# konnpaku-youmu/Model_Predictive_Control

Measured on AMD Instinct MI355X. Metric: QP solves/sec (batch, horizon N=20) at 1/2/4/8 MI355X; max|u-u_ref|, higher is better.
Workload: dtype f64; 1 GPU; cfg2: per-instance condense + box QP, FHC.py double integrator (ts=0.5), N=20, |u|<=1, x0~U(-10,10)^2; horizon=20, nx=2, nu=1, mode=fused, batch_per_gpu=4096, parallelism=dp1, graph=True, graph_steps=8, config=2

## Files before the change

model_predictive_control_amd/csrc/gi_box_core.hpp:

```cpp
#pragma once
#include <type_traits>

#include "quad.hpp"

namespace mpcqp {

template <int BS>
struct BoxOcc {
  static constexpr int w = BS <= 3 ? 4 : (BS <= 5 ? 2 : 1);
};

#ifndef MPCQP_KEYED_REDUCE
#define MPCQP_KEYED_REDUCE 1
#endif
template <class Mat>
struct QKeyed {
  static constexpr bool v = false;
};
template <int BS>
struct QKeyed<QSym<double, BS>> {
  static constexpr bool v = MPCQP_KEYED_REDUCE != 0;
};

template <class Mat>
// ... 7 lines not shown
  static constexpr int oZ = oUb + NV;
  static constexpr int oEnd = oZ + (QKeyed<Mat>::v ? NV : 0);
};

template <typename T>
__device__ __forceinline__ T bound_scale(T bnd) {
  return finite(bnd) ? T(1) / (T(1) + fabs(bnd)) : __builtin_nan("");
}

template <typename T, int RO>
struct QBounds {
  T lo[RO], hi[RO], sl[RO], su[RO];
  __device__ __forceinline__ void load(const int (&mi)[RO], const T* lbs, const T* ubs) {
#pragma unroll
    for (int s = 0; s < RO; ++s) {
      lo[s] = lbs[mi[s]];
      hi[s] = ubs[mi[s]];
      sl[s] = bound_scale(lo[s]);
      su[s] = bound_scale(hi[s]);
    }
  }
};

constexpr int key_bits(int nmax) {
  int b = 0;
  while ((1 << b) < nmax) ++b;
  return b;
}
template <int KB>
struct Key {
  static constexpr long long MASK = (1ll << KB) - 1;
  static __device__ __forceinline__ double clear(double v) {
    return __longlong_as_double(__double_as_longlong(v) & ~MASK);
  }
  static __device__ __forceinline__ double pack(double v, int code) {
    return __longlong_as_double((__double_as_longlong(v) & ~MASK) | (long long)(unsigned)code);
  }
  static __device__ __forceinline__ int code(double key) {
    return (int)(__double_as_longlong(key) & MASK);
  }
  static __device__ __forceinline__ double big() {
    return __longlong_as_double(0x7fefffffffffffffll & ~MASK);
  }
};
#ifndef MPCQP_KEY_BARE
#define MPCQP_KEY_BARE 1
#endif
__device__ __forceinline__ double key_max(double a, double b) {
#if MPCQP_KEY_BARE
  double r;
  asm("v_max_f64 %0, %1, %2" : "=v"(r) : "v"(a), "v"(b));
  return r;
#else
  return fmax(a, b);
#endif
}
__device__ __forceinline__ double key_min(double a, double b) {
#if MPCQP_KEY_BARE
  double r;
  asm("v_min_f64 %0, %1, %2" : "=v"(r) : "v"(a), "v"(b));
  return r;
#else
  return fmin(a, b);
#endif
}
template <bool MAX, int CTRL>
__device__ __forceinline__ void key_step(double& key) {
  const double o = dpp<CTRL>(key);
  key = MAX ? key_max(key, o) : key_min(key, o);
}

#ifndef MPCQP_ROW_OWNER
#define MPCQP_ROW_OWNER 1
#endif
template <class Mat>
struct QRowOwned {
  static constexpr bool v = false;
};
template <typename T, int BS>
struct QRowOwned<QSym<T, BS>> {
  static constexpr bool v = MPCQP_ROW_OWNER != 0;
};

template <class Mat_, bool OWN_ROWS = QRowOwned<Mat_>::v, bool KEY = true>
struct RowOwn {
  using Mat = Mat_;
  static constexpr bool OWNED = false;
  static constexpr bool KEYED = false;
  static constexpr int BS = Mat::RPL;
  static constexpr int RO = BS;
  static __device__ __forceinline__ bool has(const Mat&, int) { return true; }
  static __device__ __forceinline__ int row(const Mat& M, int s) { return M.bi * BS + s; }
  static __device__ __forceinline__ int mrow(const Mat& M, int s) { return M.bi * BS + s; }
  template <bool MAX, typename T, typename... P>
  static __device__ __forceinline__ void arg(T& v, int& idx, P&... pay) {
    Mat::template rows_arg<MAX>(v, idx, pay...);
  }
  template <typename T>
  static __device__ __forceinline__ T column(Mat& M, int k, T* gb, T (&colr)[BS],
                                             T (&colc)[Mat::NC], T (&cown)[RO]) {
    const T d = M.column(k, gb, colr, colc);
#pragma unroll
    for (int r = 0; r < BS; ++r) cown[r] = colr[r];
    return d;
  }
  template <typename T>
  static __device__ __forceinline__ void matvec(Mat& M, const T (&w)[RO], T* gb, T (&out)[RO]) {
    M.matvec(w, gb, out);
  }
};

template <class Mat_, bool KEY>
struct RowOwn<Mat_, true, KEY> {
  using Mat = Mat_;
  static constexpr bool OWNED = true;
  static constexpr int BS = Mat::RPL;
  static constexpr int RO = Mat::RO;
  static __device__ __forceinline__ bool has(const Mat& M, int s) { return M.owns(s); }
  static __device__ __forceinline__ int row(const Mat& M, int s) {
    return M.owns(s) ? M.bi * BS + M.own_row(s) : -1;
  }
  static __device__ __forceinline__ int mrow(const Mat& M, int s) {
    return M.bi * BS + M.own_mrow(s);
  }
  template <typename X>
  static __device__ __forceinline__ void deal(const Mat& M, const X (&full)[BS], X pad,
                                              X (&own)[RO]) {
#pragma unroll
    for (int s = 0; s < RO; ++s) {
      own[s] = pad;
#pragma unroll
      for (int j = 0; j < 4; ++j)
        if (4 * s + j < BS) own[s] = (M.bj == j) ? full[4 * s + j] : own[s];
    }
  }
  template <typename X>
  static __device__ __forceinline__ void gather(const Mat&, const X (&own)[RO], X (&full)[BS]) {
#pragma unroll
    for (int r = 0; r < BS; ++r) {
      const X v = own[r / 4];
      full[r] = (r % 4 == 0)   ? quad_lane<0>(v)
                : (r % 4 == 1) ? quad_lane<1>(v)
                : (r % 4 == 2) ? quad_lane<2>(v)
                               : quad_lane<3>(v);
    }
  }
  template <bool MAX, typename T, typename... P>
  static __device__ __forceinline__ void arg(T& v, int& idx, P&... pay) {
    Mat::template group_arg<MAX>(v, idx, pay...);
  }
  static constexpr bool KEYED = KEY && QKeyed<Mat>::v;
  using K = Key<key_bits(Mat::NMAX)>;
  template <bool MAX>
  static __device__ __forceinline__ void key_arg(double& key) {
    key_step<MAX, 0xB1>(key);
    key_step<MAX, 0x4E>(key);
    key_step<MAX, 0x124>(key);
    key_step<MAX, 0x128>(key);
  }
  template <typename T>
  static __device__ __forceinline__ T column(Mat& M, int k, T* gb, T (&colr)[BS],
                                             T (&colc)[Mat::NC], T (&cown)[RO]) {
    return M.column(k, gb, colr, colc, cown);
  }
  template <typename T>
  static __device__ __forceinline__ void matvec(Mat& M, const T (&w)[RO], T* gb, T (&out)[RO]) {
    M.matvec_own(w, gb, out);
  }
};

template <bool OWNED, class A, class B>
__device__ __forceinline__ auto& own_or_full(A& own, B& full) {
  if constexpr (OWNED) return own;
  else return full;
}


template <typename T>
__device__ __forceinline__ T mu_rate(int st, T cs, T sgn) {
  return ((st == 1) ? -cs : ((st == 2) ? cs : T(0))) * sgn;
}

template <class Own, typename T>
struct SelCmp {
  static constexpr int RO = Own::RO;
  const int (&ri)[RO];
  __device__ __forceinline__ SelCmp(const int (&ri_)[RO], const int (&)[RO], T*) : ri(ri_) {}
  __device__ __forceinline__ void scan(const int (&st)[RO], const T (&zr)[RO],
                                       const QBounds<T, RO>& B, T& viol, int& pi, T& zv) const {
    viol = -Lim<T>::inf();
    pi = 0;
    zv = T(0);
#pragma unroll
    for (int r = 0; r < RO; ++r) {
      const T vl = (B.lo[r] - zr[r]) * B.sl[r];
      const T vu = (zr[r] - B.hi[r]) * B.su[r];
      const T v = (st[r] == 0) ? fmax(vl, vu) : -Lim<T>::inf();
      const bool take = v > viol;
      viol = take ? v : viol;
      pi = take ? ri[r] : pi;
      zv = take ? zr[r] : zv;
    }
    Own::template arg<true>(viol, pi, zv);
  }
  __device__ __forceinline__ bool release(const int (&st)[RO], const T (&mu)[RO], T tol,
                                          int& k) const {
    T mv = Lim<T>::inf();
#pragma unroll
    for (int r = 0; r < RO; ++r) {
      const bool a = (st[r] == 1 || st[r] == 2) && mu[r] < -tol;
      const bool take = a && mu[r] < mv;
      mv = take ? mu[r] : mv;
      k = take ? ri[r] : k;
    }
    Own::template arg<false>(mv, k);
    return mv < Lim<T>::inf();
  }
  __device__ __forceinline__ void ratio(const int (&st)[RO], const T (&mu)[RO],
                                        const T (&co)[RO], T rm, T sgn, T& ti, int& k) const {
    ti = Lim<T>::inf();
#pragma unroll
    for (int r = 0; r < RO; ++r) {
      const T dmu = mu_rate(st[r], co[r] * rm, sgn);
      const bool cand = (st[r] == 1 || st[r] == 2) && dmu < T(0);
      const T t = cand ? -mu[r] * fast_rcp(dmu) : Lim<T>::inf();
      const bool take = t < ti;
      ti = take ? t : ti;
      k = take ? ri[r] : k;
    }
    Own::template arg<false>(ti, k);
  }
  template <class Mat>
  __device__ __forceinline__ void publish(const Mat&, const T (&)[RO]) const {}
  __device__ __forceinline__ T pivot_z(int, T zv) const { return zv; }
};

template <class Own>
struct SelKey {
  static constexpr int RO = Own::RO;
  using Mat = typename Own::Mat;
  using K = typename Own::K;
  int mi[RO], cmax[RO];
  double* zs;
  __device__ __forceinline__ SelKey(const int (&)[RO], const int (&mi_)[RO], double* gb)
      : zs(gb + BoxLds<Mat>::oZ) {
#pragma unroll
    for (int r = 0; r < RO; ++r) {
      mi[r] = mi_[r];
      cmax[r] = int(K::MASK) - mi_[r];
    }
  }
  __device__ __forceinline__ void scan(const int (&st)[RO], const double (&zr)[RO],
                                       const QBounds<double, RO>& B, double& viol, int& pi,
                                       double&) const {
    double key = -K::big();
#pragma unroll
    for (int r = 0; r < RO; ++r) {
      const double vl = (B.lo[r] - zr[r]) * B.sl[r];
      const double vu = (zr[r] - B.hi[r]) * B.su[r];
      const double v = fmin(fmax(fmax(vl, vu), -K::big()), K::big());
      key = key_max(key, K::pack((st[r] == 0) ? v : -K::big(), cmax[r]));
    }
    Own::template key_arg<true>(key);
    viol = K::clear(key);
    pi = int(K::MASK) - K::code(key);
  }
  __device__ __forceinline__ bool release(const int (&st)[RO], const double (&mu)[RO],
                                          double tol, int& k) const {
    double key = K::big();
#pragma unroll
    for (int r = 0; r < RO; ++r) {
      const bool a = (st[r] == 1 || st[r] == 2) && mu[r] < -tol;
      key = key_min(key, K::pack(a ? fmax(mu[r], -K::big()) : K::big(), cmax[r]));
    }
    Own::template key_arg<false>(key);
    k = int(K::MASK) - K::code(key);
    return K::clear(key) < K::big();
  }
  __device__ __forceinline__ void ratio(const int (&st)[RO], const double (&mu)[RO],
                                        const double (&co)[RO], double rm, double sgn,
                                        double& ti, int& k) const {
    double key = K::big();
#pragma unroll
    for (int r = 0; r < RO; ++r) {
      const double dmu = mu_rate(st[r], co[r] * rm, sgn);
      const bool cand = (st[r] == 1 || st[r] == 2) && dmu < 0.0;
      const double t = cand ? fmin(-mu[r] * fast_rcp(dmu), K::big()) : K::big();
      key = key_min(key, K::pack(t, mi[r]));
    }
    Own::template key_arg<false>(key);
    ti = K::clear(key);
    k = K::code(key);
  }
  __device__ __forceinline__ void publish(const Mat& M, const double (&zr)[RO]) const {
#pragma unroll
    for (int r = 0; r < RO; ++r)
      if (Own::has(M, r)) zs[mi[r]] = zr[r];
  }
  __device__ __forceinline__ double pivot_z(int p, double) const { return zs[p]; }
};

template <bool WARM, class Own_ = void, class Mat, typename T>
__device__ __forceinline__ int gi_box_st(Mat& M, T* gb, const T* fs, const T* lbs,
                                         const T* ubs, int n, int max_iter, T tol, bool live,
                                         T (&zfull)[Mat::RPL], int& iters,
                                         int (&stfull)[Mat::RPL] MPCQP_CLK_PARAM) {
  using Own = std::conditional_t<std::is_void_v<Own_>, RowOwn<Mat>, Own_>;
  static_assert(std::is_same_v<typename Own::Mat, Mat>, "policy of another layout");
  constexpr int BS = Mat::RPL, NC = Mat::NC;
  constexpr int RO = Own::RO;
  int ri[RO], mi[RO];
#pragma unroll
  for (int r = 0; r < RO; ++r) {
    ri[r] = Own::row(M, r);
    mi[r] = Own::mrow(M, r);
  }
  QBounds<T, RO> B;
  B.load(mi, lbs, ubs);
  const std::conditional_t<Own::KEYED, SelKey<Own>, SelCmp<Own, T>> sel(ri, mi, gb);
  T zown[Own::OWNED ? RO : 1], mu[RO];
  int stown[Own::OWNED ? RO : 1];
  auto& zr = own_or_full<Own::OWNED>(zown, zfull);
  auto& st = own_or_full<Own::OWNED>(stown, stfull);
  if constexpr (WARM && Own::OWNED) Own::deal(M, stfull, 3, stown);
#pragma unroll
  for (int r = 0; r < RO; ++r) {
    if constexpr (!WARM) st[r] = (Own::has(M, r) && ri[r] < n) ? 0 : 3;
    mu[r] = T(0);
    zr[r] = T(0);
  }
  iters = 0;
  int code = MPCQP_STATUS_OPTIMAL;
  auto refresh = [&]() {
    T w[RO], s[RO];
#pragma unroll
    for (int r = 0; r < RO; ++r) {
      const T zA = (st[r] == 1) ? B.lo[r] : ((st[r] == 2) ? B.hi[r] : T(0));
      w[r] = (st[r] == 0) ? fs[mi[r]] : -zA;
      zr[r] = zA;
    }
    Own::matvec(M, w, gb, s);
#pragma unroll
    for (int r = 0; r < RO; ++r) {
      const T g = fs[mi[r]] - s[r];
      zr[r] = (st[r] == 0) ? s[r] : zr[r];
      mu[r] = (st[r] == 1) ? g : ((st[r] == 2) ? -g : T(0));
    }
    sel.publish(M, zr);
  };
  refresh();
  bool active = live;
  if constexpr (WARM) {
    bool drop = live;
    while (true) {
      int k = 0;
      const bool found = sel.release(st, mu, tol, k);
      drop = drop && found;
      if (!__any(drop)) break;
      if (drop && ++iters > max_iter) {
        code = MPCQP_STATUS_MAXITER;
        drop = false;
        active = false;
      }
      T kr[BS], kc[NC];
      const T d = M.column(k, gb, kr, kc);
      if (drop && !(d > T(0))) {
        code = MPCQP_STATUS_NOT_CONVEX;
        drop = false;
        active = false;
      }
      if (drop) {
        M.sweep_col(k, T(1), d, kr, kc);
#pragma unroll
        for (int r = 0; r < RO; ++r)
          if (ri[r] == k) st[r] = 0;
      }
      refresh();
    }
  }
  for (int pass = 0; pass < 3; ++pass) {
    bool need_p = true;
    int p = 0, side = 1;
    T tgt = T(0), zp = T(0), gp = T(0);
    T a_viol = T(0), a_zv = T(0);
    int a_pi = 0;
    bool have_scan = false;
    while (true) {
      if (__any(active && need_p)) {
        T viol, zv = T(0);
        int pi;
        if (have_scan) {
          viol = a_viol;
          pi = a_pi;
          zv = a_zv;
        } else {
          sel.scan(st, zr, B, viol, pi, zv);
        }
        if (active && need_p) {
          if (!(viol > tol)) {
            active = false;
          } else {
            p = pi;
            const T lbp = lbs[p], ubp = ubs[p];
            zp = sel.pivot_z(p, zv);
            side = (zp < lbp) ? 1 : 2;
            tgt = (side == 1) ? lbp : ubp;
            gp = T(0);
            need_p = false;
          }
        }
      }
      MPCQP_PHASE(5);
      if (!__any(active)) break;
      bool stepping = active;
      if (stepping && ++iters > max_iter) {
        code = MPCQP_STATUS_MAXITER;
        active = false;
        stepping = false;
      }
      T c[BS], cc[NC], co[RO];
      const T mpp = Own::column(M, p, gb, c, cc, co);
      const T rm = fast_rcp(mpp);
      const T sgn = (tgt > zp) ? T(1) : T(-1);
      const T t2 = fabs(tgt - zp);
      T ti;
      int k = 0;
      sel.ratio(st, mu, co, rm, sgn, ti, k);
      const bool partial = ti < t2;
      const T s_eff = stepping ? (partial ? ti : t2) : T(0);
#pragma unroll
      for (int r = 0; r < RO; ++r) {
        const T cs = co[r] * rm;
        zr[r] = (st[r] == 0) ? fma(sgn * s_eff, cs, zr[r]) : zr[r];
        mu[r] = fma(s_eff, mu_rate(st[r], cs, sgn), mu[r]);
      }
      gp = fma(-sgn * s_eff, rm, gp);
      zp = fma(sgn, s_eff, zp);
      MPCQP_PHASE(6);
      const int idx = partial ? k : p;
      const T sigma = partial ? T(1) : T(-1);
      T kr[BS], kcol[NC];
      T d = mpp;
      if (__any(stepping && partial)) {
        d = M.column(idx, gb, kr, kcol);
      } else {
#pragma unroll
        for (int r = 0; r < BS; ++r) kr[r] = c[r];
#pragma unroll
        for (int r = 0; r < NC; ++r) kcol[r] = cc[r];
      }
      const bool bad = stepping && (partial ? !(d > T(0)) : !(d < T(0)));
      if (stepping && !bad) {
#pragma unroll
        for (int r = 0; r < RO; ++r) {
          const int i = ri[r];
          if (partial && i == k) {
            st[r] = 0;
            mu[r] = T(0);
          }
          if (!partial && i == p) {
            st[r] = side;
            zr[r] = tgt;
            mu[r] = (side == 1) ? gp : -gp;
          }
        }
        need_p = !partial;
      }
      if (bad) {
        code = MPCQP_STATUS_NOT_CONVEX;
        active = false;
      }
      sel.publish(M, zr);
      sel.scan(st, zr, B, a_viol, a_pi, a_zv);
      have_scan = true;
      if (stepping && !bad) M.sweep_col(idx, sigma, d, kr, kcol);
      MPCQP_PHASE(7);
    }
    refresh();
    T viol, zv = T(0);
    int pi;
    sel.scan(st, zr, B, viol, pi, zv);
    active = live && code == MPCQP_STATUS_OPTIMAL && viol > tol;
    if (!__any(active)) break;
  }
#pragma unroll
  for (int r = 0; r < RO; ++r) {
    zr[r] = fmin(fmax(zr[r], B.lo[r]), B.hi[r]);
  }
  if constexpr (Own::OWNED) {
    Own::gather(M, zown, zfull);
    Own::gather(M, stown, stfull);
  }
  return code;
}

template <class Own = void, class Mat, typename T>
__device__ __forceinline__ int gi_box(Mat& M, T* gb, const T* fs, const T* lbs, const T* ubs,
                                      int n, int max_iter, T tol, bool live,
                                      T (&zr)[Mat::RPL], int& iters MPCQP_CLK_PARAM) {
  int st[Mat::RPL];
  return gi_box_st<false, Own>(M, gb, fs, lbs, ubs, n, max_iter, tol, live, zr, iters,
                               st MPCQP_CLK_ARG);
}

template <typename T, int BS>
__device__ __forceinline__ int gi_box_core(Sym2D<T, BS>& M, T* buf, const T* fs, const T* lbs,
                                           const T* ubs, int n, int max_iter, T tol,
                                           T (&zr)[BS], int& iters) {
#ifdef MPCQP_PHASE_TIMING
  PhaseClock mpcqp_clk;
#endif
  return gi_box(M, buf, fs, lbs, ubs, n, max_iter, tol, true, zr, iters MPCQP_CLK_ARG);
}

}
```

model_predictive_control_amd/csrc/loop_box.hip:

```cpp
#include <type_traits>

#include "box_vjp_core.hpp"
#include "gi_box_core.hpp"
#include "quad_api.hpp"

namespace mpcqp {

template <typename T>
struct LoopArgs {
  int batch, nx, nu, N, n, steps;
  const T* H; int64_t sH;
  const T* F; int64_t sF;
  const T* A; int64_t sA;
  const T* B; int64_t sB;
  const T* x0; int64_t sX0;
  const T* lb; int64_t slb;
  const T* ub; int64_t sub;
  T* xs;
  T* us;
  T* zs;
  int32_t* status;
  int max_iter;
  T tol;
};

template <typename T>
struct LoopAffineArgs : LoopArgs<T> {
  const T* g; int64_t sG, gT;
  const T* w;
  int cold;
};

template <typename T, bool AFFINE>
using LoopArgsOf = std::conditional_t<AFFINE, LoopAffineArgs<T>, LoopArgs<T>>;

template <typename T, int NX, int NU, int BS>
struct LoopLds {
  using Box = BoxLds<QSym<T, BS>>;
  static constexpr int NMAX = 4 * BS;
  static constexpr int PMAX = NMAX * (NMAX + 1) / 2;
  static constexpr int oP = Box::oEnd;
  static constexpr int oF = oP + PMAX;
  static constexpr int oA = oF + NMAX * NX;
  static constexpr int oB = oA + NX * NX;
  static constexpr int oX = oB + NX * NU;
  static constexpr int oU = oX + NX;
  static constexpr int oS = oU + NU;
  static constexpr int size = oS + NMAX;
};

template <typename T, int BS>
struct LoopOcc {
  static constexpr int w = BS <= 2 ? 4 : 1;
};

template <typename T, int NX, int NU, int BS, bool AFFINE>
struct LoopKeyed {
  static constexpr bool v = !(sizeof(T) == 8 && NX == 4 && NU == 2 && BS == 5 && AFFINE);
};

template <typename T>
using GlobalPtr = const __attribute__((address_space(1))) T*;
template <typename T>
__device__ __forceinline__ GlobalPtr<T> sbase(const T* p) {
  const unsigned long long v = (unsigned long long)p;
  const unsigned lo = (unsigned)__builtin_amdgcn_readfirstlane((int)(v & 0xffffffffull));
  const unsigned hi = (unsigned)__builtin_amdgcn_readfirstlane((int)(v >> 32));
  return (GlobalPtr<T>)(((unsigned long long)hi << 32) | lo);
}

template <typename T>
__device__ __forceinline__ T at_bytes(GlobalPtr<T> base, unsigned bytes) {
  return *(GlobalPtr<T>)((const __attribute__((address_space(1))) char*)base + bytes);
}

template <typename T>
__device__ __forceinline__ void put_at(T* base, int64_t row, unsigned off, T v) {
  const unsigned long long p = (unsigned long long)(base + row);
  const unsigned lo = (unsigned)__builtin_amdgcn_readfirstlane((int)(p & 0xffffffffull));
  const unsigned hi = (unsigned)__builtin_amdgcn_readfirstlane((int)(p >> 32));
  asm volatile("" : "+v"(off));
  *(__attribute__((address_space(1))) T*)((__attribute__((address_space(1))) char*)(
        ((unsigned long long)hi << 32) | lo) + off * (unsigned)sizeof(T)) = v;
}

template <typename T, int NX, int NU, int BS, bool AFFINE = false>
__global__ __launch_bounds__(64, (LoopOcc<T, BS>::w)) void box_loop_kernel(
    LoopArgsOf<T, AFFINE> a) {
  using Lq = LoopLds<T, NX, NU, BS>;
  using Box = BoxLds<QSym<T, BS>>;
  constexpr int NMAX = Lq::NMAX;
  extern __shared__ __attribute__((aligned(16))) char smem_raw[];
  const int lane = threadIdx.x, g = lane >> 4, q = lane & 15;
  const int b = blockIdx.x * 4 + g;
  [[maybe_unused]] const int64_t b0 = (int64_t)blockIdx.x * 4;
  const bool live = b < a.batch;
  const int bl = live ? b : 0;
  const int n = a.n, nx = a.nx, nu = a.nu, P = n * (n + 1) / 2;
  T* gs = reinterpret_cast<T*>(smem_raw) + g * Lq::size;
  T* gb = gs + Box::oBuf;
  T* fs = gs + Box::oF;
  T* lbs = gs + Box::oLb;
  T* ubs = gs + Box::oUb;
  T* Ps = gs + Lq::oP;
  T* Fs = gs + Lq::oF;
  T* As = gs + Lq::oA;
  T* Bs = gs + Lq::oB;
  T* xg = gs + Lq::oX;
  T* ug = gs + Lq::oU;
  T* sg = gs + Lq::oS;

  {
    const T* Hb = a.H + (int64_t)bl * a.sH;
    for (int e = q; e < Lq::PMAX; e += 16) Ps[e] = e < P ? Hb[e] : T(0);
    const T* Fb = a.F + (int64_t)bl * a.sF;
    for (int e = q; e < NMAX * NX; e += 16) {
      const int i = e / NX, j = e - i * NX;
      Fs[e] = (i < n && j < nx) ? Fb[i * nx + j] : T(0);
    }
    for (int e = q; e < NX * NX; e += 16) {
      const int i = e / NX, j = e - i * NX;
      As[e] = (i < nx && j < nx) ? a.A[(int64_t)bl * a.sA + i * nx + j] : T(0);
    }
    for (int e = q; e < NX * NU; e += 16) {
      const int i = e / NU, j = e - i * NU;
      Bs[e] = (i < nx && j < nu) ? a.B[(int64_t)bl * a.sB + i * nu + j] : T(0);
    }
    if (q < NX) xg[q] = q < nx ? a.x0[(int64_t)bl * a.sX0 + q] : T(0);
  }
  bool nonfinite = false, badbox = false;
  for (int i = q; i < NMAX; i += 16) {
    const bool v = live && i < n;
    const T li = (v && a.lb) ? a.lb[(int64_t)b * a.slb + i] : -Lim<T>::inf();
    const T ui = (v && a.ub) ? a.ub[(int64_t)b * a.sub + i] : Lim<T>::inf();
    lbs[i] = li;
    ubs[i] = ui;
    badbox |= v && (!(li <= ui) || li == Lim<T>::inf() || ui == -Lim<T>::inf());
  }
  __syncthreads();
  for (int e = q; e < P; e += 16) nonfinite |= live && !finite(Ps[e]);
  for (int e = q; e < NMAX * NX; e += 16) nonfinite |= live && !finite(Fs[e]);
// ... 10 lines not shown
  M.init(lane);
  int st[BS];
#pragma unroll
  for (int r = 0; r < BS; ++r) st[r] = (M.bi * BS + r < n) ? 0 : 3;
  int failed = MPCQP_STATUS_OPTIMAL;
  int okst[BS];
#pragma unroll
  for (int r = 0; r < BS; ++r) {
    const int i = M.bi * BS + r;
    okst[r] = (lbs[i] > -Lim<T>::inf() ? 1 : 0) | (ubs[i] < Lim<T>::inf() ? 2 : 0);
  }

  constexpr bool WPACK = BS <= 2;
  [[maybe_unused]] T gn0 = T(0), gn1 = T(0), wn = T(0);
  [[maybe_unused]] auto fetch_g = [&](int t) {
    if constexpr (AFFINE) {
      if (live && a.g) {
        const auto gt = sbase(a.g + (int64_t)t * a.gT + b0 * a.sG);
        unsigned o = a.sG ? (unsigned)(g * n + q) : (unsigned)q;
        asm volatile("" : "+v"(o));
        if (q < n) gn0 = at_bytes(gt, o * (unsigned)sizeof(T));
        if constexpr (NMAX > 16)
          if (q + 16 < n) gn1 = at_bytes(gt, (o + 16u) * (unsigned)sizeof(T));
      }
    }
  };
  [[maybe_unused]] auto fetch_w = [&](int t) {
    if constexpr (AFFINE) {
      const int j = WPACK ? q - 8 : q;
      if (live && a.w && j >= 0 && j < nx) {
        const auto wt = sbase(a.w + ((int64_t)t * a.batch + b0) * nx);
        unsigned o = (unsigned)(g * nx + j);
        asm volatile("" : "+v"(o));
        (WPACK ? gn0 : wn) = at_bytes(wt, o * (unsigned)sizeof(T));
      }
    }
  };
  if constexpr (AFFINE)
    if (a.steps > 0) {
      fetch_g(0);
      fetch_w(0);
    }

  for (int t = 0; t < a.steps; ++t) {
    if constexpr (AFFINE) {
      if (live && q < nx) put_at(a.xs, ((int64_t)t * a.batch + b0) * nx, (unsigned)(g * nx + q), xg[q]);
    } else {
      if (live && q < nx) a.xs[((int64_t)t * a.batch + b) * nx + q] = xg[q];
    }
    bool nfx = false;
#pragma unroll
    for (int j = 0; j < NX; ++j) nfx |= !finite(xg[j]);
    if constexpr (AFFINE) {
#ifdef MPCQP_BOX_LOOP_PLAIN_LOAD
      if (t > 0) fetch_g(t);
#endif
      nfx |= (__ballot((!finite(gn0) && !(WPACK && q >= 8)) || !finite(gn1)) & gmask) != 0;
    }
    for (int i = q; i < NMAX; i += 16) {
      T s = T(0);
#pragma unroll
      for (int j = 0; j < NX; ++j) s = fma(Fs[i * NX + j], xg[j], s);
      if constexpr (AFFINE) s += i < 16 ? gn0 : gn1;
      fs[i] = s;
    }
    lds_exchange();
#ifndef MPCQP_BOX_LOOP_PLAIN_LOAD
    if constexpr (AFFINE)
      if (t + 1 < a.steps) fetch_g(t + 1);
#endif
    bool nf = false;
    M.load_packed(Ps, n, nf);
    const unsigned fmask = free_row_mask(M, st, g);
    int code = nfx ? MPCQP_STATUS_NONFINITE : code0;
    if (failed != MPCQP_STATUS_OPTIMAL) code = failed;
    const int sweeps = __popc(fmask);
    const bool okp = sweep_free_rows(M, gb, fmask, [&](int k, T d, const T(&colr)[BS],
                                                       const T(&colc)[BS]) {
      M.sweep_col(k, T(1), d, colr, colc);
    });
    if (code == MPCQP_STATUS_OPTIMAL && !okp) code = MPCQP_STATUS_NOT_CONVEX;
    T zr[BS];
    int iters = 0;
    using Own = RowOwn<QSym<T, BS>, QRowOwned<QSym<T, BS>>::v, LoopKeyed<T, NX, NU, BS, AFFINE>::v>;
    const int c2 = gi_box_st<true, Own>(M, gb, fs, lbs, ubs, n, a.max_iter, a.tol,
                                        live && code == MPCQP_STATUS_OPTIMAL, zr, iters,
                                        st MPCQP_CLK_ARG);
    if (code == MPCQP_STATUS_OPTIMAL) code = c2;
    const bool okc = code == MPCQP_STATUS_OPTIMAL || code == MPCQP_STATUS_MAXITER;
    if (!okc) {
      failed = code;
#pragma unroll
      for (int r = 0; r < BS; ++r) zr[r] = __builtin_nan("");
    }
    if (M.bj == 0) {
#pragma unroll
      for (int r = 0; r < BS; ++r) {
        const int i = M.bi * BS + r;
        if (i < NU) ug[i] = zr[r];
        if (i < NMAX) sg[i] = (T)st[r];
        if constexpr (AFFINE) {
          if (live && a.zs && i < n)
            put_at(a.zs, ((int64_t)t * a.batch + b0) * n, (unsigned)(g * n + i), zr[r]);
        } else {
          if (live && a.zs && i < n) a.zs[((int64_t)t * a.batch + b) * n + i] = zr[r];
        }
      }
    }
    const int word = (code & 0xff) | (((iters + sweeps) & 0xffff) << 8);
    if constexpr (AFFINE) {
      if (live && q == 0) put_at(a.status, (int64_t)t * a.batch + b0, (unsigned)g, (int32_t)word);
    } else {
      if (live && q == 0) a.status[(int64_t)t * a.batch + b] = word;
    }
    lds_exchange();
    if constexpr (AFFINE) {
      if (live && q < nu) put_at(a.us, ((int64_t)t * a.batch + b0) * nu, (unsigned)(g * nu + q), ug[q]);
    } else {
      if (live && q < nu) a.us[((int64_t)t * a.batch + b) * nu + q] = ug[q];
    }
    T xn = T(0);
    if (q < NX) {
#pragma unroll
      for (int j = 0; j < NX; ++j) xn = fma(As[q * NX + j], xg[j], xn);
#pragma unroll
      for (int j = 0; j < NU; ++j) xn = fma(Bs[q * NU + j], ug[j], xn);
    }
#ifdef MPCQP_BOX_LOOP_PLAIN_LOAD
    if constexpr (AFFINE)
      if (t > 0) fetch_w(t);
#endif
    if constexpr (AFFINE) xn += WPACK ? dpp<0x128>(gn0) : wn;
#ifndef MPCQP_BOX_LOOP_PLAIN_LOAD
    if constexpr (AFFINE)
      if (t + 1 < a.steps) fetch_w(t + 1);
#endif
#pragma unroll
    for (int r = 0; r < BS; ++r) {
      const int i = M.bi * BS + r;
      const int src = i + nu < n ? i + nu : i;
      const int s = okc ? ((int)sg[src] & okst[r]) : 0;
      if constexpr (AFFINE)
        st[r] = i < n && !a.cold ? s : (i < n ? 0 : 3);
      else
        st[r] = i < n ? s : 3;
    }
    lds_exchange();
    if (q < NX) xg[q] = xn;
    lds_exchange();
  }
  if constexpr (AFFINE) {
    if (live && q < nx)
      put_at(a.xs, ((int64_t)a.steps * a.batch + b0) * nx, (unsigned)(g * nx + q), xg[q]);
  } else {
    if (live && q < nx) a.xs[((int64_t)a.steps * a.batch + b) * nx + q] = xg[q];
  }
}

template <typename T, int NX, int NU, int BS, bool AFFINE>
static int launch_loop(const LoopArgsOf<T, AFFINE>& a, hipStream_t st) {
  using Lq = LoopLds<T, NX, NU, BS>;
  const size_t bytes = (size_t)4 * Lq::size * sizeof(T);
  if (bytes > 64 * 1024) {
    hipError_t e = hipFuncSetAttribute((const void*)box_loop_kernel<T, NX, NU, BS, AFFINE>,
                                       hipFuncAttributeMaxDynamicSharedMemorySize, (int)bytes);
    if (e != hipSuccess) return hip_fail(e, "hipFuncSetAttribute(box_loop)");
  }
// ... 95 lines not shown
```

model_predictive_control_amd/csrc/quad.hpp:

```cpp
#pragma once
#include "sym2d.hpp"

namespace mpcqp {

template <typename T>
__device__ __forceinline__ T quad_sum(T v) {
  v += dpp<0xB1>(v);
  v += dpp<0x4E>(v);
  return v;
}
template <int J, typename X>
__device__ __forceinline__ X quad_lane(X v) {
  return dpp<J | (J << 2) | (J << 4) | (J << 6)>(v);
}

template <typename T, int BS>
struct QSym {
  static constexpr int NMAX = 4 * BS;
  static constexpr int NV = NMAX;
  static constexpr int NC = BS;
  static constexpr int RPL = BS;
  static constexpr int CBUF = NMAX * BS;
  static constexpr int BUF = CBUF + NMAX;
  T m[BS][BS];
  int bi, bj;

  __device__ __forceinline__ void init(int lane) {
    const int q = lane & 15;
    bi = q >> 2;
    bj = q & 3;
  }

  template <bool MAX, typename... P>
  static __device__ __forceinline__ void rows_arg(T& v, int& idx, P&... pay) {
    arg_step<MAX, Dpp<0x124>>(v, idx, pay...);
    arg_step<MAX, Dpp<0x128>>(v, idx, pay...);
  }
  template <bool MAX, typename... P>
  static __device__ __forceinline__ void group_arg(T& v, int& idx, P&... pay) {
    arg_step<MAX, Dpp<0xB1>>(v, idx, pay...);
    arg_step<MAX, Dpp<0x4E>>(v, idx, pay...);
    rows_arg<MAX>(v, idx, pay...);
  }

  __device__ __forceinline__ void load_dense_sym(const T* D, int ld, int n) {
#pragma unroll
    for (int r = 0; r < BS; ++r)
#pragma unroll
      for (int c = 0; c < BS; ++c) {
        const int i = bi * BS + r, j = bj * BS + c;
        m[r][c] = (i < n && j < n) ? T(0.5) * (D[i * ld + j] + D[j * ld + i]) : T(0);
      }
  }

  __device__ __forceinline__ void load_packed(const T* Ps, int n, bool& nonfinite) {
#pragma unroll
    for (int r = 0; r < BS; ++r)
#pragma unroll
      for (int c = 0; c < BS; ++c) {
        const int i = bi * BS + r, j = bj * BS + c;
        T v = T(0);
        if (i < n && j < n) {
          const int idx = (j <= i) ? i * (i + 1) / 2 + j : j * (j + 1) / 2 + i;
          v = Ps[idx];
          nonfinite |= !finite(v);
        }
        m[r][c] = v;
      }
  }

  static constexpr int RO = (BS + 3) / 4;
  __device__ __forceinline__ int own_row(int s) const { return 4 * s + bj; }
  __device__ __forceinline__ bool owns(int s) const { return own_row(s) < BS; }
  __device__ __forceinline__ int own_mrow(int s) const {
    return own_row(s) < BS ? own_row(s) : BS - 1;
  }

  __device__ __forceinline__ T column(int k, T* gb, T (&colr)[BS], T (&colc)[BS]) {
    T unused[RO];
    return column(k, gb, colr, colc, unused);
  }
  __device__ __forceinline__ T column(int k, T* gb, T (&colr)[BS], T (&colc)[BS],
                                      T (&cown)[RO]) {
    const int kb = k / BS, kc = k - kb * BS;
    if (bj == kb) {
#pragma unroll
      for (int r = 0; r < BS; ++r)
#pragma unroll
        for (int c = 0; c < BS; ++c) gb[(bi * BS + r) * BS + c] = m[r][c];
    }
    lds_exchange();
#pragma unroll
    for (int r = 0; r < BS; ++r) colr[r] = gb[(bi * BS + r) * BS + kc];
#pragma unroll
    for (int c = 0; c < BS; ++c) colc[c] = gb[(bj * BS + c) * BS + kc];
#pragma unroll
    for (int s = 0; s < RO; ++s) cown[s] = gb[(bi * BS + own_mrow(s)) * BS + kc];
    const T d = gb[k * BS + kc];
    lds_exchange();
    return d;
  }

  __device__ __forceinline__ void sweep_col(int k, T sigma, T d, const T (&colr)[BS],
                                            const T (&colc)[BS]) {
    const T rd = fast_rcp(d);
    T a[BS], scol[BS], srow[BS];
    bool ik[BS], jk[BS];
#pragma unroll
    for (int r = 0; r < BS; ++r) {
      a[r] = colr[r] * rd;
      scol[r] = sigma * a[r];
      ik[r] = (bi * BS + r == k);
    }
#pragma unroll
    for (int c = 0; c < BS; ++c) {
      jk[c] = (bj * BS + c == k);
      srow[c] = jk[c] ? -rd : sigma * colc[c] * rd;
    }
#pragma unroll
    for (int r = 0; r < BS; ++r)
#pragma unroll
      for (int c = 0; c < BS; ++c) {
        const T gen = fma(-a[r], colc[c], m[r][c]);
        m[r][c] = ik[r] ? srow[c] : (jk[c] ? scol[r] : gen);
      }
  }

  __device__ __forceinline__ T sweep(int k, T sigma, T* gb) {
    T colr[BS], colc[BS];
    const T d = column(k, gb, colr, colc);
    sweep_col(k, sigma, d, colr, colc);
    return d;
  }

  __device__ __forceinline__ void matvec(const T (&w)[BS], T* gb, T (&out)[BS]) {
    T* wb = gb + CBUF;
    if (bj == 0) {
#pragma unroll
      for (int r = 0; r < BS; ++r) wb[bi * BS + r] = w[r];
    }
    lds_exchange();
    T wc[BS];
#pragma unroll
    for (int c = 0; c < BS; ++c) wc[c] = wb[bj * BS + c];
#pragma unroll
    for (int r = 0; r < BS; ++r) {
      T s = T(0);
#pragma unroll
      for (int c = 0; c < BS; ++c) s = fma(m[r][c], wc[c], s);
      out[r] = quad_sum(s);
    }
    lds_exchange();
  }

  __device__ __forceinline__ void matvec_own(const T (&w)[RO], T* gb, T (&out)[RO]) {
    T* wb = gb + CBUF;
#pragma unroll
    for (int s = 0; s < RO; ++s)
      if (owns(s)) wb[bi * BS + own_row(s)] = w[s];
    lds_exchange();
    T wc[BS];
#pragma unroll
    for (int c = 0; c < BS; ++c) wc[c] = wb[bj * BS + c];
#pragma unroll
    for (int s = 0; s < RO; ++s) out[s] = T(0);
#pragma unroll
    for (int r = 0; r < BS; ++r) {
      T s = T(0);
#pragma unroll
      for (int c = 0; c < BS; ++c) s = fma(m[r][c], wc[c], s);
      s = quad_sum(s);
      out[r / 4] = (bj == r % 4) ? s : out[r / 4];
    }
    lds_exchange();
  }
};

}
```

model_predictive_control_amd/csrc/quad_box.hip:

```cpp
#include "mpc_factor.hpp"
#include "gi_box_core.hpp"
#include "quad_api.hpp"

namespace mpcqp {

template <typename T, int BS>
struct QuadOcc {
  static constexpr int w = sizeof(T) == 8 ? (BS <= 3 ? 4 : (BS == 4 ? 3 : (BS == 5 ? 2 : 1)))
                                           : (BS <= 3 ? 4 : (BS <= 5 ? 3 : 2));
};

template <typename T, int BS>
__global__ __launch_bounds__(64, (QuadOcc<T, BS>::w)) void box_quad_kernel(BoxArgsQ<T> a) {
#ifdef MPCQP_PHASE_TIMING
  PhaseClock mpcqp_clk;
#endif
  using L = BoxLds<QSym<T, BS>>;
  constexpr int NMAX = L::NMAX;
  constexpr int PMAX = NMAX * (NMAX + 1) / 2;
  constexpr int GSZ = L::oEnd + PMAX;
  extern __shared__ __attribute__((aligned(16))) char smem_raw[];
  const int lane = threadIdx.x, g = lane >> 4, q = lane & 15;
  const int b = blockIdx.x * 4 + g;
  const bool live = b < a.batch;
// ... 1 lines not shown
  const int n = a.n, P = n * (n + 1) / 2;
  T* gs = reinterpret_cast<T*>(smem_raw) + g * GSZ;
  T* gb = gs + L::oBuf;
  T* fs = gs + L::oF;
  T* lbs = gs + L::oLb;
  T* ubs = gs + L::oUb;
  T* Ps = gs + L::oEnd;
  {
    constexpr int MAXT = (PMAX + 15) / 16;
    const T* Hb = a.H + (int64_t)bl * a.sH;
    T tmp[MAXT];
#pragma unroll
    for (int t = 0; t < MAXT; ++t) {
      const int e = q + 16 * t;
      tmp[t] = (e < P) ? Hb[e] : T(0);
    }
#pragma unroll
    for (int t = 0; t < MAXT; ++t) {
      const int e = q + 16 * t;
      if (e < P) Ps[e] = tmp[t];
    }
  }
  bool nonfinite = false, badbox = false;
  for (int i = q; i < NMAX; i += 16) {
    const bool v = live && i < n;
    const T fi = v ? a.f[(int64_t)b * a.sf + i] : T(0);
    const T li = (v && a.lb) ? a.lb[(int64_t)b * a.slb + i] : -Lim<T>::inf();
    const T ui = (v && a.ub) ? a.ub[(int64_t)b * a.sub + i] : Lim<T>::inf();
    fs[i] = fi;
    lbs[i] = li;
    ubs[i] = ui;
    nonfinite |= v && !finite(fi);
    badbox |= v && (!(li <= ui) || li == Lim<T>::inf() || ui == -Lim<T>::inf());
  }
  __syncthreads();
  QSym<T, BS> M;
  M.init(lane);
  M.load_packed(Ps, n, nonfinite);
  const unsigned long long gmask = 0xFFFFull << (16 * g);
  const bool g_nonfinite = (__ballot(nonfinite) & gmask) != 0;
  const bool g_badbox = (__ballot(badbox) & gmask) != 0;
  int code = MPCQP_STATUS_OPTIMAL;
  if (g_nonfinite) code = MPCQP_STATUS_NONFINITE;
  else if (g_badbox) code = MPCQP_STATUS_INFEASIBLE;
  bool ok = true;
  for (int k = 0; k < n; ++k) {
    const T d = M.sweep(k, T(1), gb);
    ok &= d > T(0);
  }
  if (code == MPCQP_STATUS_OPTIMAL && !ok) code = MPCQP_STATUS_NOT_CONVEX;
  T zr[BS];
  int iters = 0;
  const int c2 = gi_box(M, gb, fs, lbs, ubs, n, a.max_iter, a.tol,
                        live && code == MPCQP_STATUS_OPTIMAL, zr, iters MPCQP_CLK_ARG);
  if (code == MPCQP_STATUS_OPTIMAL) code = c2;
  if (code != MPCQP_STATUS_OPTIMAL && code != MPCQP_STATUS_MAXITER) {
#pragma unroll
    for (int r = 0; r < BS; ++r) zr[r] = __builtin_nan("");
  }
  if (live && M.bj == 0) {
#pragma unroll
    for (int r = 0; r < BS; ++r) {
      const int i = M.bi * BS + r;
      if (i < n) a.z[(int64_t)b * n + i] = zr[r];
    }
  }
  if (live && q == 0) a.status[b] = (code & 0xff) | ((iters & 0xffff) << 8);
}

template <typename T, int NX, int NU, int BS>
struct QMpcRows {
  static constexpr bool v = NX <= 2 && !(sizeof(T) == 8 && NU == 2 && BS <= 3);
};

template <typename T, int NX, int NU, class Mat>
struct QMpcOwned {
  static constexpr bool v =
      QRowOwned<Mat>::v && !(sizeof(T) == 8 && NX == 4 && NU == 2 && Mat::RPL == 5);
};

template <typename T, int NX, int NU, class Mat>
struct QMpcKeyed {
  static constexpr bool v = !(sizeof(T) == 8 && NX == 4 && NU == 2 && Mat::RPL == 4);
};

template <typename T, int NX, int NU, class Mat>
struct QMpcLds {
  static constexpr bool ROWS = QMpcRows<T, NX, NU, Mat::RPL>::v;
  int oA, oB, oQ, oQf, oR, oC, oX0, oK, oSi, oAcl, oX, oW, total, ld;
  __host__ __device__ QMpcLds(int N, int n, int tv) {
    const int S = tv ? N : 1;
    const int N2 = ROWS ? 0 : N;
    oA = BoxLds<Mat>::oEnd;
    oB = oA + S * NX * NX;
    oQ = oB + S * NX * NU;
    oQf = oQ + NX * NX;
    oR = oQf + NX * NX;
    oC = oR + NU * NU;
    oX0 = oC + N * NX;
    oK = oX0 + NX;
    oSi = oK + N2 * NU * NX;
    oAcl = oSi + N2 * NU * NU;
    oX = oAcl + N2 * NX * NX;
    oW = oX + (ROWS ? 0 : (N + 1) * NX);
    ld = Mat::NV + 1;
    total = (oW + n * ld + 1) & ~1;
  }
};

template <typename T, int NX, int NU>
__device__ __forceinline__ void load_sq(const T* s, T (&m)[NX][NU], int ld) {
#pragma unroll
  for (int i = 0; i < NX; ++i)
#pragma unroll
    for (int j = 0; j < NU; ++j) m[i][j] = s[i * ld + j];
}

template <typename T, int NX, int BS>
struct QMpcOcc {
  static constexpr int w = NX <= 2 ? QuadOcc<T, BS>::w : (QuadOcc<T, BS>::w < 2 ? 1 : 2);
};

#ifdef MPCQP_WAVE_CLOCK
constexpr int kWaveClockMax = 16384;
__device__ unsigned long long mpcqp_wave_clock[3 * kWaveClockMax];
#endif

template <typename T, int NX, int NU, class Mat, int GL, int OCC>
__global__ __launch_bounds__(64, OCC) void mpc_group_kernel(MpcArgsQ<T> a) {
#ifdef MPCQP_WAVE_CLOCK
  const unsigned long long wclk0 = __builtin_amdgcn_s_memrealtime();
#endif
  using BL = BoxLds<Mat>;
  constexpr int NV = BL::NV;
  constexpr int RPL = Mat::RPL;
  constexpr int GPW = kWave / GL;
  extern __shared__ __attribute__((aligned(16))) char smem_raw[];
  const int lane = threadIdx.x, g = lane / GL, q = lane % GL;
  const int b = blockIdx.x * GPW + g;
  const bool live = b < a.batch;
  const int bl = live ? b : 0;
  const int nx = a.nx, nu = a.nu, N = a.N, n = N * nu, tv = a.tv;
  const int S = tv ? N : 1;
  const QMpcLds<T, NX, NU, Mat> L(N, n, tv);
  T* sm = reinterpret_cast<T*>(smem_raw) + g * L.total;
  T* gb = sm + BL::oBuf;
  T* fs = sm + BL::oF;
  T* lbs = sm + BL::oLb;
  T* ubs = sm + BL::oUb;
  T* As = sm + L.oA;
  T* Bs = sm + L.oB;
  T* Qs = sm + L.oQ;
  T* Qfs = sm + L.oQf;
  T* Rs = sm + L.oR;
  T* Cs = sm + L.oC;
  T* X0s = sm + L.oX0;
  constexpr bool ROWS = QMpcRows<T, NX, NU, RPL>::v;
  [[maybe_unused]] T* Ks = sm + L.oK;
  [[maybe_unused]] T* Sis = sm + L.oSi;
  [[maybe_unused]] T* Acls = sm + L.oAcl;
  [[maybe_unused]] T* Xs = sm + L.oX;
  T* Wt = sm + L.oW;
  const int ld = L.ld;

#ifdef MPCQP_PHASE_TIMING
  PhaseClock mpcqp_clk;
// ... 440 lines not shown
#pragma unroll
          for (int ch = 0; ch < NCH; ++ch) {
            const bool at = t == cj[ch];
            T v[NU], u[NU], xn[NX];
#pragma unroll
            for (int i = 0; i < NU; ++i) {
              v[i] = at ? lj[ch][i] : T(0);
              T s = v[i];
#pragma unroll
              for (int qq = 0; qq < NX; ++qq) s = fma(Kt[i][qq], wx[ch][qq], s);
              u[i] = s;
            }
#pragma unroll
            for (int i = 0; i < NX; ++i) {
              T s = T(0);
#pragma unroll
              for (int qq = 0; qq < NX; ++qq) s = fma(Act[i][qq], wx[ch][qq], s);
#pragma unroll
              for (int qq = 0; qq < NU; ++qq) s = fma(Br[i][qq], v[qq], s);
              xn[i] = s;
            }
#pragma unroll
            for (int qq = 0; qq < NX; ++qq) wx[ch][qq] = xn[qq];
            if (cv[ch]) {
#pragma unroll
              for (int i = 0; i < NU; ++i)
                if (i < nu) Wc[ch][t * nu + i] = u[i];
            }
          }
        }
        if (q == 0) {
#pragma unroll
          for (int u = 0; u < NU; ++u) {
            T s = T(0);
#pragma unroll
            for (int qq = 0; qq < NX; ++qq) s = fma(Ba[qq][u], yk[qq], s);
            if (u < nu) fs[k * nu + u] = s;
          }
        }
        if (k > 0) {
          T yn[NX];
#pragma unroll
          for (int i = 0; i < NX; ++i) {
            T s = T(0);
#pragma unroll
            for (int qq = 0; qq < NX; ++qq) s = fma(Qr[i][qq], xnext[qq], s);
#pragma unroll
            for (int qq = 0; qq < NX; ++qq) s = fma(Ar[qq][i], yk[qq], s);
            yn[i] = s;
          }
#pragma unroll
          for (int qq = 0; qq < NX; ++qq) yk[qq] = yn[qq];
        }
#pragma unroll
        for (int i = 0; i < NU; ++i)
#pragma unroll
          for (int qq = 0; qq < NX; ++qq) Kt[i][qq] = Kn[i][qq];
#pragma unroll
        for (int i = 0; i < NX; ++i)
#pragma unroll
          for (int qq = 0; qq < NX; ++qq) Act[i][qq] = Acn[i][qq];
#pragma unroll
        for (int qq = 0; qq < NX; ++qq) xnext[qq] = xnn[qq];
      }
#pragma unroll
      for (int ch = 0; ch < NCH; ++ch)
        if (cv[ch])
          for (int i = n; i < NV; ++i) Wc[ch][i] = T(0);
    }
  }
  __syncthreads();

  MPCQP_PHASE(2);
  Mat M;
  M.init(lane);
  neg_gram<T>(M, Wt, ld, n);
  MPCQP_PHASE(3);
  for (int i = q; i < n; i += GL) nonfinite |= !finite(fs[i]);
  const unsigned long long gmask = (GL == 64 ? ~0ull : ((1ull << GL) - 1)) << (GL * g);
  if ((__ballot(nonfinite) & gmask) != 0) code = MPCQP_STATUS_NONFINITE;
  else if ((__ballot(badbox) & gmask) != 0) code = MPCQP_STATUS_INFEASIBLE;
  T zr[RPL];
  int iters = 0;
  using Own = RowOwn<Mat, QMpcOwned<T, NX, NU, Mat>::v, QMpcKeyed<T, NX, NU, Mat>::v>;
  const int c2 = gi_box<Own>(M, gb, fs, lbs, ubs, n, a.max_iter, a.tol,
                             live && code == MPCQP_STATUS_OPTIMAL, zr, iters MPCQP_CLK_ARG);
  if (code == MPCQP_STATUS_OPTIMAL) code = c2;
  MPCQP_PHASE(4);
#ifdef MPCQP_PHASE_TIMING
  mpcqp_clk.flush();
#endif
  if (code != MPCQP_STATUS_OPTIMAL && code != MPCQP_STATUS_MAXITER) {
#pragma unroll
    for (int r = 0; r < RPL; ++r) zr[r] = __builtin_nan("");
  }
  if (live && M.bj == 0) {
#pragma unroll
    for (int r = 0; r < RPL; ++r) {
      const int i = M.bi * RPL + r;
      if (i < n) a.z[(int64_t)b * n + i] = zr[r];
    }
  }
  if (live && q == 0) a.status[b] = (code & 0xff) | ((iters & 0xffff) << 8);
#ifdef MPCQP_WAVE_CLOCK
  {
    int itmax = 0;
#pragma unroll
    for (int gg = 0; gg < GPW; ++gg) {
      const int v = __builtin_amdgcn_readlane(iters, gg * GL);
      itmax = v > itmax ? v : itmax;
    }
    const unsigned long long wclk1 = __builtin_amdgcn_s_memrealtime();
    if (lane == 0 && blockIdx.x < kWaveClockMax) {
      mpcqp_wave_clock[3 * blockIdx.x] = wclk0;
      mpcqp_wave_clock[3 * blockIdx.x + 1] = wclk1;
      mpcqp_wave_clock[3 * blockIdx.x + 2] = (unsigned long long)itmax;
    }
  }
#endif
}

template <typename T, int BS>
int launch_box_quad(const BoxArgsQ<T>& a, hipStream_t st) {
  using L = BoxLds<QSym<T, BS>>;
  constexpr int NMAX = L::NMAX;
  const size_t bytes = (size_t)4 * (L::oEnd + NMAX * (NMAX + 1) / 2) * sizeof(T);
  hipLaunchKernelGGL((box_quad_kernel<T, BS>), dim3((a.batch + 3) / 4), dim3(kWave), bytes, st, a);
  MPCQP_CHECK_LAUNCH("box_quad_kernel");
  return MPCQP_OK;
}

template <typename T>
int solve_box_quad(const BoxArgsQ<T>& a, hipStream_t st) {
  return dispatch_bs<4>(a.n, [&](auto bs) {
    return launch_box_quad<T, decltype(bs)::value>(a, st);
  });
}

template <typename T, int NX, int NU, class Mat, int GL, int OCC>
int launch_mpc_group(const MpcArgsQ<T>& a, hipStream_t st) {
  constexpr int GPW = kWave / GL;
  const int n = a.N * a.nu;
  const QMpcLds<T, NX, NU, Mat> L(a.N, n, a.tv);
  const size_t bytes = (size_t)GPW * L.total * sizeof(T);
  if (bytes > 160 * 1024) {
    set_error("mpcqp_mpc_box: LDS footprint %zu B > 160 KiB", bytes);
    return MPCQP_ENOTSUP;
  }
  auto kern = mpc_group_kernel<T, NX, NU, Mat, GL, OCC>;
  if (bytes > 64 * 1024) {
    hipError_t e = hipFuncSetAttribute((const void*)kern,
                                       hipFuncAttributeMaxDynamicSharedMemorySize, (int)bytes);
    if (e != hipSuccess) return hip_fail(e, "hipFuncSetAttribute(mpc_group)");
  }
  hipLaunchKernelGGL(kern, dim3((a.batch + GPW - 1) / GPW), dim3(kWave), bytes, st, a);
  MPCQP_CHECK_LAUNCH("mpc_group_kernel");
  return MPCQP_OK;
}

template <typename T, int NX, int NU, int BS>
int launch_mpc_quad(const MpcArgsQ<T>& a, hipStream_t st) {
  return launch_mpc_group<T, NX, NU, QSym<T, BS>, 16, QMpcOcc<T, NX, BS>::w>(a, st);
}

template <typename T, int NX, int NU>
int mpc_quad_bs(const MpcArgsQ<T>& a, hipStream_t st) {
  return dispatch_bs<4>(a.N * a.nu, [&](auto bs) {
// ... 31 lines not shown
```

Measured before the change: 91.52 million solves/s.

## Add fast full-step path, prefetch next pivot bounds, defer sweep with precomputed reciprocal

Splits the dual active-set inner step into two variants. A cheap conservative filter decides whether any active constraint could block the step, and when none can, a full-step variant skips the keyed ratio reduction and the column fetch. The bounds and z value for the next pivot are prefetched right after the violation scan, and the rank-1 sweep is deferred past the branch using the already-computed reciprocal. This adds the filter's per-row work and extra live registers, and the filter tolerance could misjudge near-ties.

```diff
diff --git a/model_predictive_control_amd/csrc/gi_box_core.hpp b/model_predictive_control_amd/csrc/gi_box_core.hpp
--- a/model_predictive_control_amd/csrc/gi_box_core.hpp
+++ b/model_predictive_control_amd/csrc/gi_box_core.hpp
@@ -113,11 +113,22 @@
   static constexpr bool v = MPCQP_ROW_OWNER != 0;
 };
 
-template <class Mat_, bool OWN_ROWS = QRowOwned<Mat_>::v, bool KEY = true>
+#ifndef MPCQP_FAST_TRIP
+#define MPCQP_FAST_TRIP 1
+#endif
+#ifndef MPCQP_BOUND_AHEAD
+#define MPCQP_BOUND_AHEAD 1
+#endif
+#ifndef MPCQP_SWEEP_RD
+#define MPCQP_SWEEP_RD 1
+#endif
+
+template <class Mat_, bool OWN_ROWS = QRowOwned<Mat_>::v, bool KEY = true, bool TRIP = true>
 struct RowOwn {
   using Mat = Mat_;
   static constexpr bool OWNED = false;
   static constexpr bool KEYED = false;
+  static constexpr bool FAST = false, AHEAD = false, SWEEP_RD = false;
   static constexpr int BS = Mat::RPL;
   static constexpr int RO = BS;
   static __device__ __forceinline__ bool has(const Mat&, int) { return true; }
@@ -141,8 +152,8 @@
   }
 };
 
-template <class Mat_, bool KEY>
-struct RowOwn<Mat_, true, KEY> {
+template <class Mat_, bool KEY, bool TRIP>
+struct RowOwn<Mat_, true, KEY, TRIP> {
   using Mat = Mat_;
   static constexpr bool OWNED = true;
   static constexpr int BS = Mat::RPL;
@@ -181,6 +192,9 @@
     Mat::template group_arg<MAX>(v, idx, pay...);
   }
   static constexpr bool KEYED = KEY && QKeyed<Mat>::v;
+  static constexpr bool FAST = TRIP && (KEYED ? MPCQP_FAST_TRIP != 0 : MPCQP_FAST_TRIP == 2);
+  static constexpr bool AHEAD = TRIP && (KEYED ? MPCQP_BOUND_AHEAD != 0 : MPCQP_BOUND_AHEAD == 2);
+  static constexpr bool SWEEP_RD = FAST && MPCQP_SWEEP_RD != 0;
   using K = Key<key_bits(Mat::NMAX)>;
   template <bool MAX>
   static __device__ __forceinline__ void key_arg(double& key) {
@@ -210,6 +224,35 @@
 template <typename T>
 __device__ __forceinline__ T mu_rate(int st, T cs, T sgn) {
   return ((st == 1) ? -cs : ((st == 2) ? cs : T(0))) * sgn;
+}
+
+template <typename T>
+struct RatioFilter;
+template <>
+struct RatioFilter<double> {
+  static constexpr double DELTA = 0x1p-40, TINY = 0x1p-900;
+};
+template <>
+struct RatioFilter<float> {
+  static constexpr float DELTA = 0x1p-16f, TINY = 0x1p-100f;
+};
+template <typename T>
+__device__ __forceinline__ bool ratio_range(T t2, T huge) {
+  return t2 >= RatioFilter<T>::TINY && t2 <= huge;
+}
+template <typename T, int RO>
+__device__ __forceinline__ bool ratio_filter(const int (&st)[RO], const T (&mu)[RO],
+                                             const T (&co)[RO], T rm, T sgn, T t2) {
+  const T t2d = t2 * (T(1) + RatioFilter<T>::DELTA);
+  bool f = false;
+#pragma unroll
+  for (int r = 0; r < RO; ++r) {
+    const T dmu = mu_rate(st[r], co[r] * rm, sgn);
+    const bool cand = (st[r] == 1 || st[r] == 2) && dmu < T(0);
+    const T rhs = t2d * -dmu;
+    f = f || (cand && (mu[r] < rhs || rhs < RatioFilter<T>::TINY));
+  }
+  return f;
 }
 
 template <class Own, typename T>
@@ -261,6 +304,10 @@
     }
     Own::template arg<false>(ti, k);
   }
+  __device__ __forceinline__ bool may_block(const int (&st)[RO], const T (&mu)[RO],
+                                            const T (&co)[RO], T rm, T sgn, T t2) const {
+    return ratio_filter(st, mu, co, rm, sgn, t2) || !ratio_range(t2, Lim<T>::inf());
+  }
   template <class Mat>
   __device__ __forceinline__ void publish(const Mat&, const T (&)[RO]) const {}
   __device__ __forceinline__ T pivot_z(int, T zv) const { return zv; }
@@ -322,6 +369,11 @@
     Own::template key_arg<false>(key);
     ti = K::clear(key);
     k = K::code(key);
+  }
+  __device__ __forceinline__ bool may_block(const int (&st)[RO], const double (&mu)[RO],
+                                            const double (&co)[RO], double rm, double sgn,
+                                            double t2) const {
+    return ratio_filter(st, mu, co, rm, sgn, t2) || !ratio_range(t2, K::big());
   }
   __device__ __forceinline__ void publish(const Mat& M, const double (&zr)[RO]) const {
 #pragma unroll
@@ -415,6 +467,7 @@
     T tgt = T(0), zp = T(0), gp = T(0);
     T a_viol = T(0), a_zv = T(0);
     int a_pi = 0;
+    [[maybe_unused]] T a_lb = T(0), a_ub = T(0), a_zp = T(0);
     bool have_scan = false;
     while (true) {
       if (__any(active && need_p)) {
@@ -432,10 +485,17 @@
             active = false;
           } else {
             p = pi;
-            const T lbp = lbs[p], ubp = ubs[p];
-            zp = sel.pivot_z(p, zv);
-            side = (zp < lbp) ? 1 : 2;
-            tgt = (side == 1) ? lbp : ubp;
+            if constexpr (Own::AHEAD) {
+              const T lbp = have_scan ? a_lb : lbs[p], ubp = have_scan ? a_ub : ubs[p];
+              zp = have_scan ? a_zp : sel.pivot_z(p, zv);
+              side = (zp < lbp) ? 1 : 2;
+              tgt = (side == 1) ? lbp : ubp;
+            } else {
+              const T lbp = lbs[p], ubp = ubs[p];
+              zp = sel.pivot_z(p, zv);
+              side = (zp < lbp) ? 1 : 2;
+              tgt = (side == 1) ? lbp : ubp;
+            }
             gp = T(0);
             need_p = false;
           }
@@ -454,57 +514,25 @@
       const T rm = fast_rcp(mpp);
       const T sgn = (tgt > zp) ? T(1) : T(-1);
       const T t2 = fabs(tgt - zp);
-      T ti;
-      int k = 0;
-      sel.ratio(st, mu, co, rm, sgn, ti, k);
-      const bool partial = ti < t2;
-      const T s_eff = stepping ? (partial ? ti : t2) : T(0);
-#pragma unroll
-      for (int r = 0; r < RO; ++r) {
-        const T cs = co[r] * rm;
-        zr[r] = (st[r] == 0) ? fma(sgn * s_eff, cs, zr[r]) : zr[r];
-        mu[r] = fma(s_eff, mu_rate(st[r], cs, sgn), mu[r]);
-      }
-      gp = fma(-sgn * s_eff, rm, gp);
-      zp = fma(sgn, s_eff, zp);
-      MPCQP_PHASE(6);
-      const int idx = partial ? k : p;
-      const T sigma = partial ? T(1) : T(-1);
-      T kr[BS], kcol[NC];
-      T d = mpp;
-      if (__any(stepping && partial)) {
-        d = M.column(idx, gb, kr, kcol);
+      [[maybe_unused]] T s_kr[BS], s_kcol[NC], s_sigma = T(-1), s_d = mpp;
+      [[maybe_unused]] int s_idx = p;
+      [[maybe_unused]] bool sweeping = false;
+      if constexpr (!Own::FAST) {
+#define MPCQP_TRIP_FULL false
+#include "gi_box_trip.inc"
+#undef MPCQP_TRIP_FULL
+      } else if (__any(stepping && sel.may_block(st, mu, co, rm, sgn, t2))) {
+#define MPCQP_TRIP_FULL false
+#include "gi_box_trip.inc"
+#undef MPCQP_TRIP_FULL
       } else {
-#pragma unroll
-        for (int r = 0; r < BS; ++r) kr[r] = c[r];
-#pragma unroll
-        for (int r = 0; r < NC; ++r) kcol[r] = cc[r];
-      }
-      const bool bad = stepping && (partial ? !(d > T(0)) : !(d < T(0)));
-      if (stepping && !bad) {
-#pragma unroll
-        for (int r = 0; r < RO; ++r) {
-          const int i = ri[r];
-          if (partial && i == k) {
-            st[r] = 0;
-            mu[r] = T(0);
-          }
-          if (!partial && i == p) {
-            st[r] = side;
-            zr[r] = tgt;
-            mu[r] = (side == 1) ? gp : -gp;
-          }
-        }
-        need_p = !partial;
-      }
-      if (bad) {
-        code = MPCQP_STATUS_NOT_CONVEX;
-        active = false;
-      }
-      sel.publish(M, zr);
-      sel.scan(st, zr, B, a_viol, a_pi, a_zv);
-      have_scan = true;
-      if (stepping && !bad) M.sweep_col(idx, sigma, d, kr, kcol);
+#define MPCQP_TRIP_FULL true
+#include "gi_box_trip.inc"
+#undef MPCQP_TRIP_FULL
+      }
+      if constexpr (Own::FAST) {
+        if (sweeping) M.template sweep_col<Own::SWEEP_RD>(s_idx, s_sigma, s_d, s_kr, s_kcol);
+      }
       MPCQP_PHASE(7);
     }
     refresh();
diff --git a/model_predictive_control_amd/csrc/gi_box_trip.inc b/model_predictive_control_amd/csrc/gi_box_trip.inc
--- /dev/null
+++ b/model_predictive_control_amd/csrc/gi_box_trip.inc
@@ -0,0 +1,71 @@
+{
+  constexpr bool FULL = MPCQP_TRIP_FULL;
+  T ti = T(0);
+  int k = 0;
+  if (!FULL) sel.ratio(st, mu, co, rm, sgn, ti, k);
+  const bool partial = !FULL && ti < t2;
+  const T s_eff = stepping ? (partial ? ti : t2) : T(0);
+#pragma unroll
+  for (int r = 0; r < RO; ++r) {
+    const T cs = co[r] * rm;
+    zr[r] = (st[r] == 0) ? fma(sgn * s_eff, cs, zr[r]) : zr[r];
+    mu[r] = fma(s_eff, mu_rate(st[r], cs, sgn), mu[r]);
+  }
+  gp = fma(-sgn * s_eff, rm, gp);
+  zp = fma(sgn, s_eff, zp);
+  MPCQP_PHASE(6);
+  const int idx = partial ? k : p;
+  const T sigma = partial ? T(1) : T(-1);
+  T kr[BS], kcol[NC];
+  T d = mpp;
+  if (!FULL && __any(stepping && partial)) {
+    d = M.column(idx, gb, kr, kcol);
+  } else {
+#pragma unroll
+    for (int r = 0; r < BS; ++r) kr[r] = c[r];
+#pragma unroll
+    for (int r = 0; r < NC; ++r) kcol[r] = cc[r];
+  }
+  const bool bad = stepping && (partial ? !(d > T(0)) : !(d < T(0)));
+  if (stepping && !bad) {
+#pragma unroll
+    for (int r = 0; r < RO; ++r) {
+      const int i = ri[r];
+      if (partial && i == k) {
+        st[r] = 0;
+        mu[r] = T(0);
+      }
+      if (!partial && i == p) {
+        st[r] = side;
+        zr[r] = tgt;
+        mu[r] = (side == 1) ? gp : -gp;
+      }
+    }
+    need_p = !partial;
+  }
+  if (bad) {
+    code = MPCQP_STATUS_NOT_CONVEX;
+    active = false;
+  }
+  sel.publish(M, zr);
+  sel.scan(st, zr, B, a_viol, a_pi, a_zv);
+  have_scan = true;
+  if constexpr (Own::AHEAD) {
+    const int pa = a_pi < BoxLds<Mat>::NV - 1 ? a_pi : BoxLds<Mat>::NV - 1;
+    a_lb = lbs[pa];
+    a_ub = ubs[pa];
+    a_zp = sel.pivot_z(pa, a_zv);
+  }
+  if constexpr (Own::FAST) {
+    sweeping = stepping && !bad;
+    s_idx = idx;
+    s_sigma = sigma;
+#pragma unroll
+    for (int r = 0; r < BS; ++r) s_kr[r] = kr[r];
+#pragma unroll
+    for (int r = 0; r < NC; ++r) s_kcol[r] = kcol[r];
+    s_d = !Own::SWEEP_RD ? d : (FULL ? rm : fast_rcp(d));
+  } else {
+    if (stepping && !bad) M.sweep_col(idx, sigma, d, kr, kcol);
+  }
+}
diff --git a/model_predictive_control_amd/csrc/loop_box.hip b/model_predictive_control_amd/csrc/loop_box.hip
--- a/model_predictive_control_amd/csrc/loop_box.hip
+++ b/model_predictive_control_amd/csrc/loop_box.hip
@@ -57,6 +57,11 @@
 template <typename T, int NX, int NU, int BS, bool AFFINE>
 struct LoopKeyed {
   static constexpr bool v = !(sizeof(T) == 8 && NX == 4 && NU == 2 && BS == 5 && AFFINE);
+};
+
+template <typename T, int NX, int NU, int BS, bool AFFINE>
+struct LoopTrip {
+  static constexpr bool v = BS != 2;
 };
 
 template <typename T>
@@ -233,7 +238,8 @@
     if (code == MPCQP_STATUS_OPTIMAL && !okp) code = MPCQP_STATUS_NOT_CONVEX;
     T zr[BS];
     int iters = 0;
-    using Own = RowOwn<QSym<T, BS>, QRowOwned<QSym<T, BS>>::v, LoopKeyed<T, NX, NU, BS, AFFINE>::v>;
+    using Own = RowOwn<QSym<T, BS>, QRowOwned<QSym<T, BS>>::v, LoopKeyed<T, NX, NU, BS, AFFINE>::v,
+                       LoopTrip<T, NX, NU, BS, AFFINE>::v>;
     const int c2 = gi_box_st<true, Own>(M, gb, fs, lbs, ubs, n, a.max_iter, a.tol,
                                         live && code == MPCQP_STATUS_OPTIMAL, zr, iters,
                                         st MPCQP_CLK_ARG);
diff --git a/model_predictive_control_amd/csrc/quad.hpp b/model_predictive_control_amd/csrc/quad.hpp
--- a/model_predictive_control_amd/csrc/quad.hpp
+++ b/model_predictive_control_amd/csrc/quad.hpp
@@ -101,9 +101,10 @@
     return d;
   }
 
+  template <bool RD = false>
   __device__ __forceinline__ void sweep_col(int k, T sigma, T d, const T (&colr)[BS],
                                             const T (&colc)[BS]) {
-    const T rd = fast_rcp(d);
+    const T rd = RD ? d : fast_rcp(d);
     T a[BS], scol[BS], srow[BS];
     bool ik[BS], jk[BS];
 #pragma unroll
diff --git a/model_predictive_control_amd/csrc/quad_box.hip b/model_predictive_control_amd/csrc/quad_box.hip
--- a/model_predictive_control_amd/csrc/quad_box.hip
+++ b/model_predictive_control_amd/csrc/quad_box.hip
@@ -107,6 +107,11 @@
 template <typename T, int NX, int NU, class Mat>
 struct QMpcKeyed {
   static constexpr bool v = !(sizeof(T) == 8 && NX == 4 && NU == 2 && Mat::RPL == 4);
+};
+
+template <typename T, int NX, int NU, class Mat>
+struct QMpcTrip {
+  static constexpr bool v = true;
 };
 
 template <typename T, int NX, int NU, class Mat>
@@ -713,7 +718,8 @@
   else if ((__ballot(badbox) & gmask) != 0) code = MPCQP_STATUS_INFEASIBLE;
   T zr[RPL];
   int iters = 0;
-  using Own = RowOwn<Mat, QMpcOwned<T, NX, NU, Mat>::v, QMpcKeyed<T, NX, NU, Mat>::v>;
+  using Own = RowOwn<Mat, QMpcOwned<T, NX, NU, Mat>::v, QMpcKeyed<T, NX, NU, Mat>::v,
+                     QMpcTrip<T, NX, NU, Mat>::v>;
   const int c2 = gi_box<Own>(M, gb, fs, lbs, ubs, n, a.max_iter, a.tol,
                              live && code == MPCQP_STATUS_OPTIMAL, zr, iters MPCQP_CLK_ARG);
   if (code == MPCQP_STATUS_OPTIMAL) code = c2;
```

Result: faster. 96.53 million solves/s (median of 6 runs) (+5.5%).
